# XuehaiPan/mate

Hardware: AMD Instinct MI355X
Metric: env-steps/sec MATE-4v8-9 batch=4096 per GPU (random policy, auto-reset) (higher is better)
Workload: dtype f64; 1 GPU; MATE-4v8-9.yaml batch=4096 envs per GPU, uniform random policy (on-device Philox), fused 256-step launches, restarts every 1 launch(es); global_batch=4096, parallelism=env-shard x1, steps_per_launch=256

## Files before the change

include/mate_engine.h:

```cpp
#ifndef MATE_ENGINE_H
#define MATE_ENGINE_H

#include <stdint.h>

#ifdef __cplusplus
extern "C" {
#endif

#define MATE_ABI_VERSION 1

enum {
    MATE_OK = 0,
    MATE_EINVAL = -1,
    MATE_EHIP = -2,
    MATE_ENOMEM = -3,
    MATE_ESTATE = -4
};

enum { MATE_OBS_F32 = 0, MATE_OBS_F64 = 1 };
enum { MATE_ACT_F32 = 0, MATE_ACT_F64 = 1,
       MATE_ACT_CAMERA_DISCRETE = 0x100, MATE_ACT_TARGET_DISCRETE = 0x200 };

typedef struct mate_config {
    int32_t num_cameras, num_targets, num_obstacles;
// ... 157 lines not shown
    float *scalars_dev;
    void  *final_obs_dev;
} mate_first_rows;
int mate_engine_enable_first_rows(mate_engine *engine, const mate_first_rows *config);

int mate_engine_lut_read(mate_engine *engine, int64_t env, int32_t camera, double *phis_host,
                         double *rhos_host, int32_t capacity, int32_t *count);

int mate_engine_enable_outer_boundary(mate_engine *engine, int32_t *capacity);
int mate_engine_lut_read_outer(mate_engine *engine, int64_t env, int32_t camera, double *phis, double *rhos,
                               int32_t capacity, int32_t *count);
int mate_engine_lut_write_outer(mate_engine *engine, int64_t env, int32_t camera, const double *phis_host,
                                const double *rhos_host, int32_t count);
int mate_engine_soft_coverage(mate_engine *engine, const uint32_t *masks_dev, double *matrix_dev, double *scores_dev, void *stream);
int mate_engine_lut_write(mate_engine *engine, int64_t env, int32_t camera, const double *phis_host,
                          const double *rhos_host, int32_t count);
int mate_engine_rebuild_luts(mate_engine *engine, void *stream);

int mate_engine_idle_steps(mate_engine *engine, int64_t *total);

int mate_engine_kernel_time(mate_engine *engine, int32_t enable, double *avg_ms, int64_t *launches);

int mate_engine_last_flow(const mate_engine *engine);

int mate_engine_set_store_form(mate_engine *engine, int32_t shifted);
int mate_engine_block_alloc(int32_t device, int64_t bytes, void **ptr_out);
int mate_engine_block_free(void *ptr);
int mate_engine_block_probe(int32_t device, void *block, int64_t bytes, int32_t rows_per_step, int32_t row_bytes, void *stream,
                            double *gbytes_per_s);
int mate_engine_set_sub_wave(mate_engine *engine, int32_t enable, int32_t *in_use);
int mate_engine_hbm_probe(int32_t device, const void *src, void *dst, int64_t bytes, int32_t mode, void *stream, double *gbytes_per_s);
int mate_engine_memory_hold(int32_t device, int64_t bytes, void **token_out);
int mate_engine_memory_release(void *token);

#ifdef __cplusplus
}
#endif
#endif
```

mate_amd/_native.py:

```python
import ctypes
import os

__all__ = ['lib', 'load', 'EngineError', 'MateConfig', 'MateLayout', 'MateStepIO', 'MatePolicyTape', 'MateRewardRows', 'MateFragmentRows', 'MateFirstRows', 'LIB_PATH', 'check', 'EXPORTED_SYMBOLS']

LIB_PATH = os.environ.get('MATE_ENGINE_LIB') or os.path.join(os.path.dirname(os.path.abspath(__file__)), 'lib', 'libmate_engine.so')

class EngineError(RuntimeError):

    def __init__(self, code, message):
        super().__init__(f'mate_engine error {code}: {message}')
        self.code = code


class MateConfig(ctypes.Structure):
    _fields_ = [
        ('num_cameras', ctypes.c_int32), ('num_targets', ctypes.c_int32), ('num_obstacles', ctypes.c_int32),
        ('max_episode_steps', ctypes.c_int32), ('sparse_reward', ctypes.c_int32),
        ('num_cargoes_per_target', ctypes.c_int32), ('shuffle_entities', ctypes.c_int32),
        ('targets_start_with_cargoes', ctypes.c_int32),
        ('high_capacity_target_split', ctypes.c_double), ('bounty_factor', ctypes.c_double),
        ('transmittance', ctypes.c_double),
        ('camera_radius', ctypes.c_double), ('camera_min_viewing_angle', ctypes.c_double),
        ('camera_max_sight_range', ctypes.c_double), ('camera_rotation_step', ctypes.c_double),
        ('camera_zooming_step', ctypes.c_double),
# ... 83 lines not shown
    'mate_engine_export_state': (INT, [P, P, P]),
    'mate_engine_import_state': (INT, [P, P, P]),
    'mate_engine_enable_state_rows': (INT, [P, P, I32, P, P]),
    'mate_engine_state_rows': (INT, [P, P, I32, P, P, P]),
    'mate_engine_enable_reward_rows': (INT, [P, ctypes.POINTER(MateRewardRows)]),
    'mate_engine_enable_selection': (INT, [P, I32, P, P, P, P, I32]),
    'mate_engine_disable_selection': (INT, [P]),
    'mate_engine_selection_actions': (INT, [P, ctypes.POINTER(P), ctypes.POINTER(I32)]),
    'mate_engine_step_selected': (INT, [P, IO, TAPE, I32, P]),
    'mate_engine_enable_fragment_rows': (INT, [P, ctypes.POINTER(MateFragmentRows)]),
    'mate_engine_fragment_coefficients': (INT, [P, ctypes.POINTER(P), ctypes.POINTER(I32)]),
    'mate_engine_fragment_rows': (INT, [P, ctypes.POINTER(MateFragmentRows), IO, I32, P]),
    'mate_engine_enable_first_rows': (INT, [P, ctypes.POINTER(MateFirstRows)]),
    'mate_engine_lut_read': (INT, [P, I64, I32, P, P, I32, ctypes.POINTER(I32)]),
    'mate_engine_lut_read_outer': (INT, [P, I64, I32, P, P, I32, ctypes.POINTER(I32)]),
    'mate_engine_enable_outer_boundary': (INT, [P, ctypes.POINTER(I32)]),
    'mate_engine_lut_write': (INT, [P, I64, I32, P, P, I32]),
    'mate_engine_lut_write_outer': (INT, [P, I64, I32, P, P, I32]),
    'mate_engine_soft_coverage': (INT, [P, P, P, P, P]),
    'mate_engine_rebuild_luts': (INT, [P, P]),
    'mate_engine_idle_steps': (INT, [P, ctypes.POINTER(I64)]),
    'mate_engine_kernel_time': (INT, [P, I32, F64P, ctypes.POINTER(I64)]),
    'mate_engine_last_flow': (INT, [P]),
    'mate_engine_block_alloc': (INT, [I32, I64, ctypes.POINTER(P)]),
    'mate_engine_block_free': (INT, [P]),
    'mate_engine_block_probe': (INT, [I32, P, I64, I32, I32, P, F64P]),
    'mate_engine_set_store_form': (INT, [P, I32]),
    'mate_engine_memory_hold': (INT, [I32, I64, ctypes.POINTER(P)]),
    'mate_engine_memory_release': (INT, [P]),
    'mate_engine_hbm_probe': (INT, [I32, P, P, I64, I32, P, F64P]),
    'mate_engine_set_sub_wave': (INT, [P, I32, ctypes.POINTER(I32)]),
}
EXPORTED_SYMBOLS = tuple(PROTOTYPES)

lib = None


def load():
    global lib
    if lib is not None:
        return lib
    if not os.path.exists(LIB_PATH):
        raise ImportError(
            f'{LIB_PATH} is missing: build the HIP engine first (python -m mate_amd.build or '
            f'__graft_entry__.build()).  mate_amd has no CPU fallback.')
    import torch
# ... 79 lines not shown
```

mate_amd/build.py:

```python
import json
import os
import re
import subprocess
import sys

HERE = os.path.dirname(os.path.abspath(__file__))
SRC = os.path.join(HERE, 'csrc', 'mate_engine.hip')
DEPS = [SRC] + [os.path.join(HERE, 'csrc', f) for f in ('engine_kernels.hpp', 'reset_kernels.hpp', 'policy_kernels.hpp', 'aux_kernels.hpp', 'attached_tile.hpp', 'state_rows.hpp', 'reward_rows.hpp', 'fragment_rows.hpp', 'selection_rows.hpp', 'device_math.hpp', 'instrument.hpp',
                                                          'shape_groups.hpp', 'shape_group.inc', 'shape_group.hip', 'engine_host.h',
                                                          'opponent_rows.hpp', 'opponent_kernels.inc', 'opponent_kernels.hip')] + [
    os.path.join(os.path.dirname(HERE), 'include', 'mate_engine.h')]
OUT = os.path.join(HERE, 'lib', 'libmate_engine.so')
FLAGS = ['--offload-arch=gfx950', '-O3', '-std=c++17', '-ffp-contract=off', '-fPIC', '-shared',
         '-mllvm', '-disable-machine-licm']


STAMP = os.path.join(HERE, 'lib', 'build_stamp.json')


def source_digest():
    import hashlib
    h = hashlib.sha256(' '.join(FLAGS).encode())
    for d in DEPS:
        with open(d, 'rb') as fh:
            h.update(os.path.basename(d).encode() + b'\0' + fh.read())
    return h.hexdigest()


def needs_build():
    if not os.path.exists(OUT) or not os.path.exists(STAMP):
        return True
    try:
        with open(STAMP) as fh:
            return json.load(fh).get('sources') != source_digest()
    except (OSError, ValueError):
        return True


RESOURCES = os.path.join(HERE, 'lib', 'kernel_resources.json')
OPPONENT_SRC = os.path.join(HERE, 'csrc', 'opponent_kernels.hip')
OPPONENT_RESOURCES = os.path.join(HERE, 'lib', 'kernel_resources_opponents.json')
_REMARK = re.compile(r'remark:\s+(Function Name|TotalSGPRs|VGPRs|ScratchSize \[bytes/lane\]|Dynamic Stack|Occupancy \[waves/SIMD\]|SGPRs Spill|VGPRs Spill): (\S+)')


def parse_resources(text):
    kernels, current = {}, None
    for key, value in _REMARK.findall(text):
        if key == 'Function Name':
            current = kernels.setdefault(value, {})
        elif current is not None:
            current[key.split(' [')[0]] = value if key == 'Dynamic Stack' else int(value)
    return kernels


N_SHAPE_GROUPS = 6


def _compile_and_link(out, extra=(), verbose=False, remarks=False):
    import concurrent.futures
    hipcc = os.environ.get('HIPCC', '/opt/rocm/bin/hipcc')
    objdir = os.path.join(os.path.dirname(OUT), 'obj', os.path.splitext(os.path.basename(out))[0])
    os.makedirs(objdir, exist_ok=True)
    compile_flags = [f for f in FLAGS if f != '-shared'] + list(extra) + ['-DMATE_SPLIT_BUILD'] + (['-Rpass-analysis=kernel-resource-usage'] if remarks else [])
    units = [(SRC, [], os.path.join(objdir, 'mate_engine.o'))]
    units += [(os.path.join(HERE, 'csrc', 'shape_group.hip'), [f'-DMATE_SHAPE_GROUP={k}'], os.path.join(objdir, f'shape_group_{k}.o')) for k in range(N_SHAPE_GROUPS)]
    units += [(OPPONENT_SRC, [], os.path.join(objdir, 'opponent_kernels.o'))]

    def compile_unit(unit):
        src, defs, obj = unit
        cmd = [hipcc] + compile_flags + defs + ['-c', '-o', obj, src]
        if verbose:
            print(' '.join(cmd), flush=True)
        done = subprocess.run(cmd, stdout=subprocess.PIPE, stderr=subprocess.PIPE, universal_newlines=True)
        return cmd, done

    workers = max(1, min(len(units), int(os.environ.get('MATE_BUILD_JOBS', '0')) or (os.cpu_count() or 2)))
    with concurrent.futures.ThreadPoolExecutor(max_workers=workers) as pool:
        results = list(pool.map(compile_unit, units))
    text, opponent_text = '', ''
    for (src, _, _), (cmd, done) in zip(units, results):
        if done.returncode != 0:
            sys.stderr.write(done.stderr)
            raise subprocess.CalledProcessError(done.returncode, cmd)
        if src == OPPONENT_SRC:
            opponent_text += done.stderr
        else:
            text += done.stderr
    link = [hipcc, '--offload-arch=gfx950', '-shared', '-fPIC', '-o', out] + [u[2] for u in units]
    if verbose:
        print(' '.join(link), flush=True)
    done = subprocess.run(link, stdout=subprocess.PIPE, stderr=subprocess.PIPE, universal_newlines=True)
    if done.returncode != 0:
        sys.stderr.write(done.stderr)
        raise subprocess.CalledProcessError(done.returncode, link)
    return text, opponent_text


def build_engine(force=False, verbose=False):
    if not force and not needs_build():
        return OUT
    os.makedirs(os.path.dirname(OUT), exist_ok=True)
    text, opponent_text = _compile_and_link(OUT, verbose=verbose, remarks=True)
    kernels, opponents = parse_resources(text), parse_resources(opponent_text)
    for path, table in ((RESOURCES, kernels), (OPPONENT_RESOURCES, opponents)):
        with open(path, 'w') as f:
            json.dump(table, f, indent=1, sort_keys=True)
    bad = [k for k, r in list(kernels.items()) + list(opponents.items()) if r.get('ScratchSize', 0) != 0 or r.get('Dynamic Stack') != 'False']
    if bad:
        os.remove(OUT)
        raise RuntimeError('kernels with private scratch memory: ' + ', '.join(bad))
    with open(STAMP, 'w') as f:
        json.dump({'sources': source_digest()}, f)
    return OUT


def build_profiling(verbose=False):
    out = os.path.join(HERE, 'lib', 'libmate_engine_prof.so')
    _compile_and_link(out, extra=['-DMATE_PHASE_CLOCKS'], verbose=verbose)
    return out


def build_tools(verbose=False):
    hipcc = os.environ.get('HIPCC', '/opt/rocm/bin/hipcc')
    tools = os.path.join(os.path.dirname(os.path.dirname(os.path.abspath(__file__))), 'tools')
    built = []
    for name in ('store_roof', 'store_bits', 'store_contig', 'store_vmm', 'region_bw', 'valu_rates', 'chunk_order', 'dispatch_probe', 'va_reuse', 'store_layout'):
        src, out = os.path.join(tools, name + '.hip'), os.path.join(tools, name)
        if not os.path.exists(src) or (os.path.exists(out) and os.path.getmtime(out) >= os.path.getmtime(src)):
            continue
        cmd = [hipcc, '--offload-arch=gfx950', '-O3', '-std=c++17', '-I' + os.path.dirname(SRC), '-o', out, src]
# ... 23 lines not shown
```

mate_amd/csrc/engine_host.h:

```cpp
#pragma once
#include <hip/hip_runtime.h>

#include <cstdint>
#include <string>
#include <utility>
#include <vector>

#include "../../include/mate_engine.h"
#include "reset_kernels.hpp"
#include "reward_rows.hpp"
#include "fragment_rows.hpp"
#include "selection_rows.hpp"
#include "opponent_rows.hpp"
#include "state_rows.hpp"
#include "shape_groups.hpp"

using namespace mate;

constexpr size_t kLdsCeiling = 160 * 1024;

struct Switches {
    bool generic = false;
    bool flow_generic = false;
    int stagger = -1;
    int lut_small_cap = 0;
    bool reset_monolithic = false;
    int rollout_rotate = 1;
    bool no_image = false;
    bool policy_split = false;
    int step_split = -1;
    bool zoom_iterate = false;
    bool step_sub_wave = true;
    int sub_wave_mode = 2;
    bool step_greedy_rollout = false;
    bool pipelined_low_priority = true;
    bool pipelined_serial = false;
};
struct StateRows {
    void *dst = nullptr; bool f64 = false; const void *ab = nullptr; void *d_ab = nullptr, *d_ab_demand = nullptr;
    std::vector<double> demand_table;
    bool on() const { return dst != nullptr; }
};
struct RewardRows {
    bool on = false, f64 = false, soft = false, accumulate = false;
    RewardArgs args{};
    int32_t *d_snapshot = nullptr; double *d_matrix = nullptr, *d_scores = nullptr;
};
struct Selection {
    bool on = false, act_f64 = true;
    SelectionArgs args{};
    double *d_actions = nullptr;
    bool masks_stale = false;
};
struct Opponent {
    int kind = MATE_OPPONENT_GREEDY;
    double *d_final = nullptr;
    bool drifted = false;
};
struct FragmentRows {
// ... 15 lines not shown
    Params p{};
    Params *d_params = nullptr;
    Ptrs g{};
    ResetLds rl{};
    ResetLds rl_small{};
    mate_config cfg{};
    int device = 0;
    int64_t N = 0;
    int parity = 0;
    uint32_t tick = 0;
    int64_t steps_since_reset = 0;
    bool was_reset = false;
    bool dev_tick = false;
    int dev_frames = 1;
    int dev_interval = 1;
    int pending_interval = 0;
    bool pipelined = false;
    int pipe_every = 1, pipe_count = 0;
    hipStream_t side = nullptr;
    hipEvent_t ev_launch = nullptr, ev_reset[2] = {nullptr, nullptr};
    bool reset_in_flight[2] = {false, false};
    size_t step_lds = 0, reset_lds = 0;
    KernelSet k{};
    size_t image_wave_bytes = 0;
    int64_t cus = 256;
    int split_on = 0;
    int last_flow = 0;
    std::vector<void *> allocs;
    bool policy_ready = false;
    PolicyPtrs q{};
    int greedy_team_bits = 0;
    int cam_mode = 0, tgt_mode = 0;
    bool xf_relative = false, xf_cam = false, xf_tgt = false;
    std::vector<double> xf_cam_scale, xf_cam_bias, xf_tgt_scale, xf_tgt_bias;
    uint2 *d_xdesc = nullptr;
    void *d_xab = nullptr;
    Opponent opponent;
    StateRows state; RewardRows reward; Selection selection; FragmentRows fragment; FirstRows first;
    int timing = 0;
    int64_t timing_tick = 0;
    std::vector<std::pair<hipEvent_t, hipEvent_t>> events;
    size_t events_used = 0;
};

struct LaunchPlan {
    StepFn step = nullptr; PolicyFn policy = nullptr;
// ... 10 lines not shown
    if (mode == 0 || e->k.sub_wave <= 1 || !(greedy ? (const void *)e->k.rollout_greedy_sub : (const void *)e->k.rollout_sub[0])) return 1;
    if (mode == 1) return e->k.sub_wave;
    if (e->N < 32 * e->cus) return 1;
    if (!greedy && e->p.Nc * e->p.Nt >= 16) return 1;
    return e->k.sub_wave;
}
static int folded_flow(const mate_engine *e, int mode, const Ptrs &g) {
    const bool common = !e->sw.flow_generic && !g.tape_ct && !g.tape_goal && !g.act_discrete && g.obs_mode == 0 && !g.xdesc && !g.xab &&
                        g.scratch_init && (g.cam_obs || e->p.Nc == 0) && g.tgt_obs && g.scalars;
    if (common && mode == MODE_STEP_RANDOM) return FLOW_RANDOM;
    if (common && mode == MODE_STEP) return FLOW_ACT_F32;
    return FLOW_ANY;
}

static LaunchPlan plan_step(const mate_engine *e, int mode, const Ptrs &g) {
    LaunchPlan pl;
    const int flow = pl.last_flow = folded_flow(e, mode, g);
    pl.E = (mode != MODE_OBSERVE && e->sw.step_sub_wave && !e->p.obs_f64) ? sub_wave_of_launch(e, false) : 1;
    if (pl.E > 1) { pl.step = e->k.rollout_sub[flow]; pl.blocks = blocks_of(e, 4 * pl.E); pl.lds = pl.E * e->step_lds; }
    else if (e->split_on && e->k.split[flow]) { pl.step = e->k.split[flow]; pl.blocks = blocks_of(e, 1); pl.threads = 128; pl.lds = e->step_lds / 4; }
    else { pl.step = e->k.step[flow]; pl.blocks = blocks_of(e, 4); pl.lds = e->step_lds; }
    return pl;
}
static LaunchPlan plan_rollout_random(const mate_engine *e, const Ptrs &g) {
    LaunchPlan pl;
    const int flow = pl.last_flow = folded_flow(e, MODE_STEP_RANDOM, g);
    pl.E = sub_wave_of_launch(e, false);
    pl.blocks = blocks_of(e, 4 * pl.E);
    if (pl.E > 1) { pl.step = e->k.rollout_sub[flow]; pl.lds = pl.E * e->step_lds; }
    else { pl.step = e->k.rollout[flow]; pl.lds = (flow == FLOW_RANDOM && e->k.image) ? 4 * e->image_wave_bytes : e->step_lds; }
    return pl;
}
enum PolicyForm { FORM_ROLLOUT, FORM_ROLLOUT_SUB, FORM_STEP_GREEDY, kPolicyForms };
static LaunchPlan policy_form(const mate_engine *e, int form, int team_caller) {
    const Params &p = e->p;
    LaunchPlan pl;
    pl.policy = form == FORM_STEP_GREEDY ? e->k.step_greedy : form == FORM_ROLLOUT_SUB ? e->k.rollout_greedy_sub : e->k.rollout_greedy;
    pl.last_flow = form == FORM_STEP_GREEDY ? FLOW_STEP_GREEDY : FLOW_GREEDY;
    pl.E = form == FORM_ROLLOUT_SUB ? e->k.sub_wave : 1;
    pl.blocks = blocks_of(e, 4 * pl.E);
    const int slice = form == FORM_STEP_GREEDY ? step_greedy_slice_bytes(e->q.PW, e->q.TW, p.Nc, p.Nt, p.MW, team_caller != 0) : policy_slice_bytes(e->q.PW, p.Nc, p.Nt);
    pl.lds = (size_t)pl.E * (4 * (size_t)p.lds_wave_bytes + 4 * (size_t)slice) + (form != FORM_STEP_GREEDY && pl.E == 1 ? 1024 : 0);
    return pl;
}
static LaunchPlan plan_with_policies(const mate_engine *e, bool per_step, int team_caller) {
    const bool sub = (!per_step || e->sw.step_sub_wave) && sub_wave_of_launch(e, true) > 1 && policy_form(e, FORM_ROLLOUT_SUB, team_caller).fits();
    const bool light = per_step && !sub && e->k.step_greedy && !e->sw.step_greedy_rollout && policy_form(e, FORM_STEP_GREEDY, -1).fits();
    return policy_form(e, sub ? FORM_ROLLOUT_SUB : light ? FORM_STEP_GREEDY : FORM_ROLLOUT, team_caller);
}

struct Tiles { unsigned blocks = 0, threads = 256; size_t lds = 0; int E = 0; };
struct AttachedPlan {
// ... 29 lines not shown
```

mate_amd/csrc/mate_engine.hip:

```cpp
#include <hip/hip_runtime.h>
#include <hip/hip_ext.h>

#include <algorithm>
#include <atomic>
#include <cmath>
#include <cstdarg>
#include <cstdio>
#include <cstdlib>
#include <cstring>
#include <map>
#include <mutex>
#include <random>
#include <string>
#include <vector>

#include "../../include/mate_engine.h"
#include "reset_kernels.hpp"
#include "policy_kernels.hpp"
#include "aux_kernels.hpp"
#include "engine_host.h"

using namespace mate;

static thread_local std::string g_error;
// ... 12 lines not shown
        if (e_ != hipSuccess) { (void)hipGetLastError(); return fail(MATE_EHIP, "%s failed: %s", #expr, hipGetErrorString(e_)); }    \
    } while (0)

#ifndef MATE_SPLIT_BUILD
#define MATE_SHAPE_GROUP 0
#include "shape_group.inc"
#undef MATE_SHAPE_GROUP
#define MATE_SHAPE_GROUP 1
#include "shape_group.inc"
#undef MATE_SHAPE_GROUP
#define MATE_SHAPE_GROUP 2
#include "shape_group.inc"
#undef MATE_SHAPE_GROUP
#define MATE_SHAPE_GROUP 3
#include "shape_group.inc"
#undef MATE_SHAPE_GROUP
#define MATE_SHAPE_GROUP 4
#include "shape_group.inc"
#undef MATE_SHAPE_GROUP
#define MATE_SHAPE_GROUP 5
#include "shape_group.inc"
#undef MATE_SHAPE_GROUP
#include "opponent_kernels.inc"
#endif

static KernelSet pick_kernels(int Nc, int Nt, int No, bool f64, bool generic, bool no_image) {
    KernelSet k;
    if (!generic && (pick_kernels_group0(Nc, Nt, No, f64, no_image, &k) || pick_kernels_group1(Nc, Nt, No, f64, no_image, &k) ||
                     pick_kernels_group2(Nc, Nt, No, f64, no_image, &k) || pick_kernels_group3(Nc, Nt, No, f64, no_image, &k) ||
                     pick_kernels_group4(Nc, Nt, No, f64, no_image, &k) || pick_kernels_group5(Nc, Nt, No, f64, no_image, &k))) {
        k.specialised = 1;
        return k;
    }
    return f64 ? f64_kernels<AnyShape>() : f32_kernels<AnyShape, void, true>(no_image);
}

static Switches read_switches() {
    Switches w;
    auto flag = [](const char *name) { const char *v = getenv(name); return v && atoi(v) != 0; };
    w.generic = flag("MATE_GENERIC");
    w.flow_generic = flag("MATE_FLOW_GENERIC");
    if (const char *v = getenv("MATE_STAGGER")) w.stagger = atoi(v);
    if (const char *v = getenv("MATE_LUT_SMALL_CAP")) w.lut_small_cap = atoi(v);
    w.reset_monolithic = flag("MATE_RESET_MONOLITHIC");
    if (const char *v = getenv("MATE_ROLLOUT_ROTATE")) w.rollout_rotate = atoi(v);
    w.zoom_iterate = flag("MATE_ZOOM_ITERATE");
    w.policy_split = flag("MATE_POLICY_SPLIT");
    w.step_greedy_rollout = flag("MATE_STEP_GREEDY_ROLLOUT");
    w.no_image = flag("MATE_NO_IMAGE");
    if (const char *v = getenv("MATE_STEP_SUBWAVE")) w.step_sub_wave = atoi(v) != 0;
    if (const char *v = getenv("MATE_SUBWAVE")) w.sub_wave_mode = atoi(v) == 0 ? 0 : 1;
    if (const char *v = getenv("MATE_STEP_SPLIT")) w.step_split = atoi(v) != 0;
    if (const char *v = getenv("MATE_PIPELINED_PRIORITY")) w.pipelined_low_priority = atoi(v) != 0;
    w.pipelined_serial = flag("MATE_PIPELINED_SERIAL");
    return w;
}

static void note_stream(mate_engine *e, hipStream_t stream) {
    if (e->launched && stream != e->last_stream) e->multi_stream = true;
    e->last_stream = stream; e->launched = true;
}
static int leave_pipelined(mate_engine *e, hipStream_t stream);
static hipError_t wait_for_launches(mate_engine *e) {
    if (e->pipelined && leave_pipelined(e, e->last_stream) != MATE_OK) return hipErrorUnknown;
    hipError_t err = e->multi_stream ? hipErrorInvalidHandle : hipStreamSynchronize(e->last_stream);
    if (err != hipSuccess) { (void)hipGetLastError(); e->last_stream = nullptr; err = hipDeviceSynchronize(); }
    if (err == hipSuccess) { e->multi_stream = false; e->launched = false; }
    return err;
}

static int enter(mate_engine *e, hipStream_t stream, const char *who = nullptr) {
    { const int rc = leave_pipelined(e, stream); if (rc != MATE_OK) return rc; }
    if (who && !e->was_reset) return fail(MATE_ESTATE, "%s called before reset() (or import_state)", who);
    HIP_TRY(hipSetDevice(e->device));
    return MATE_OK;
}
static int enter_host(mate_engine *e) {
// ... 168 lines not shown
    e->cfg = *cfg;
    e->device = device;
    e->N = num_envs;
    Params &p = e->p;
    fill_shape(p, Nc, Nt, No, cfg->obs_dtype == MATE_OBS_F64);
    p.max_episode_steps = cfg->max_episode_steps; p.sparse_reward = cfg->sparse_reward != 0;
    p.num_cargoes_per_target = cfg->num_cargoes_per_target; p.shuffle = cfg->shuffle_entities != 0;
    p.start_with_cargoes = cfg->targets_start_with_cargoes != 0;
    p.n_high = (int)((double)Nt * std::min(std::max(cfg->high_capacity_target_split, 0.0), 1.0));
    p.tau = std::min(std::max(cfg->transmittance, 0.0), 1.0);
    p.cam_radius = cfg->camera_radius; p.theta_min = cfg->camera_min_viewing_angle; p.rmax = cfg->camera_max_sight_range;
    p.rot = cfg->camera_rotation_step; p.zoom = cfg->camera_zooming_step;
    p.area = cfg->camera_min_viewing_angle * (cfg->camera_max_sight_range * cfg->camera_max_sight_range);
    p.tgt_step = cfg->target_step_size; p.tgt_sight = cfg->target_sight_range;
    p.freight_scale = std::ceil(2000.0 / cfg->target_step_size);
    p.bounty_scale = std::ceil(p.freight_scale * std::max(0.0, cfg->bounty_factor));
    p.reward_scale = p.freight_scale + p.bounty_scale;
    p.max_team_reward = p.reward_scale * cfg->num_cargoes_per_target * Nt;
    p.obs_r_lo = cfg->obstacle_radius_range[0]; p.obs_r_hi = cfg->obstacle_radius_range[1];
    p.seed_lo = (uint32_t)seed; p.seed_hi = (uint32_t)(seed >> 32); p.first_env = (uint32_t)first_env_index;
    e->step_lds = 4 * (size_t)p.lds_wave_bytes;
    e->sw = read_switches();
    e->k = pick_kernels(Nc, Nt, No, p.obs_f64 != 0, e->sw.generic, e->sw.no_image);
    { Params pi = p; fill_shape(pi, Nc, Nt, No, false, true); e->image_wave_bytes = e->k.image ? (size_t)pi.lds_wave_bytes : (size_t)p.lds_wave_bytes; }
    if (p.lds_wave_bytes > 0xffff) { delete e; return fail(MATE_EINVAL, "scenario too large for 16-bit LDS descriptors"); }
    ResetLds &rl = e->rl;
    layout_reset_lds(p, rl, std::max(512, next_pow2(Nc > 0 ? 360 + No * 185 + 1 : 1)));
    e->reset_lds = (size_t)rl.total_bytes;
    setup_two_tier(e);
    if (e->step_lds > kLdsCeiling || e->reset_lds > kLdsCeiling) {
        const size_t a = e->step_lds, b = e->reset_lds;
        delete e;
        return fail(MATE_EINVAL, "scenario too large for the 160 KiB LDS (%zu / %zu bytes)", a, b);
    }

    int rc = MATE_OK;
    const size_t N = (size_t)num_envs;
    Ptrs &g = e->g;
    g.N = num_envs;
    {
        hipDeviceProp_t prop;
        const int64_t cus = hipGetDeviceProperties(&prop, device) == hipSuccess ? prop.multiProcessorCount : 256;
        e->cus = cus;
        const int digits = e->sw.stagger >= 0 ? e->sw.stagger : 0;

        if (e->sw.step_split < 0) e->sw.step_split = (Nc > 0 && num_envs <= 8 * cus) ? 1 : 0;
// ... 35 lines not shown
            g.scratch_init = d;
            return MATE_OK;
        });
        if (rc) break;
        std::vector<double> ranges((size_t)(Nc + No + Nt) * 4, 0.0);
        if (Nc) std::memcpy(ranges.data(), cfg->camera_location_ranges, sizeof(double) * 4 * Nc);
        if (No) std::memcpy(ranges.data() + 4 * Nc, cfg->obstacle_location_ranges, sizeof(double) * 4 * No);
        std::memcpy(ranges.data() + 4 * (Nc + No), cfg->target_location_ranges, sizeof(double) * 4 * Nt);
        double *d_ranges = nullptr;
        if ((rc = dev_alloc(e, &d_ranges, ranges.size()))) break;
        if (hipMemcpy(d_ranges, ranges.data(), ranges.size() * 8, hipMemcpyHostToDevice) != hipSuccess) { rc = fail(MATE_EHIP, "range upload failed"); break; }
        g.reset_ranges = d_ranges;
    } while (0);
    if (rc == MATE_OK) rc = dev_alloc(e, &e->d_params, (size_t)1);
    if (rc == MATE_OK) g.dev_tick_ptr = reinterpret_cast<uint32_t *>(reinterpret_cast<char *>(e->d_params) + offsetof(Params, dev_tick));
    if (rc == MATE_OK && hipMemcpy(e->d_params, &e->p, sizeof(Params), hipMemcpyHostToDevice) != hipSuccess) rc = fail(MATE_EHIP, "params upload failed");
    if (rc == MATE_OK) {
        const KernelSet &k = e->k;
        hipError_t err = hipSuccess;
        auto opt_in = [&](auto fn, size_t bytes) { if (err == hipSuccess) err = set_dynamic_lds(fn, bytes); };
        for (int f = 0; f < 3; ++f) opt_in(k.step[f], e->step_lds);
        for (int f = 0; f < 2; ++f) opt_in(k.rollout[f], f == 1 && k.image ? 4 * e->image_wave_bytes : e->step_lds);
        for (int f = 0; f < 3; ++f) opt_in(k.rollout_sub[f], k.sub_wave * e->step_lds);
        with_obs_type(p.obs_f64 != 0, [&](auto tag) { opt_in(&reset_kernel<decltype(tag)>, e->reset_lds); });
        if (err != hipSuccess) rc = fail(MATE_EHIP, "hipFuncSetAttribute failed: %s", hipGetErrorString(err));
    }
    if (rc != MATE_OK) { mate_engine_destroy(e); return rc; }
    *out = e;
    return MATE_OK;
}

extern "C" int mate_engine_destroy(mate_engine *e) {
    if (!e) return MATE_OK;
    (void)hipSetDevice(e->device);
    if (e->side) {
        (void)hipStreamSynchronize(e->side);
        (void)hipStreamDestroy(e->side);
        if (e->ev_launch) (void)hipEventDestroy(e->ev_launch);
        for (int q = 0; q < 2; ++q) if (e->ev_reset[q]) (void)hipEventDestroy(e->ev_reset[q]);
    }
    for (auto &ev : e->events) { (void)hipEventDestroy(ev.first); (void)hipEventDestroy(ev.second); }
    for (void *ptr : e->allocs) (void)hipFree(ptr);
    delete e;
    return MATE_OK;
}

// ... 743 lines not shown
extern "C" int mate_engine_step(mate_engine *e, const mate_step_io *io, int32_t auto_reset, void *stream) {
    return attached_last(e, launch_step(e, io, MODE_STEP, auto_reset, (hipStream_t)stream), (hipStream_t)stream);
}
extern "C" int mate_engine_step_random(mate_engine *e, const mate_step_io *io, int32_t auto_reset, void *stream) {
    return attached_last(e, launch_step(e, io, MODE_STEP_RANDOM, auto_reset, (hipStream_t)stream), (hipStream_t)stream);
}
static int rollout_random_impl(mate_engine *e, const mate_step_io *io, int32_t steps, int32_t auto_reset, void *stream_) {
    if (!e) return fail(MATE_EINVAL, "null engine");
    hipStream_t stream = (hipStream_t)stream_;
    { const int rc_ = enter(e, stream, "rollout"); if (rc_ != MATE_OK) return rc_; }
    if (e->dev_tick) return fail(MATE_ESTATE, "not available while the step counter is device-resident (mate_engine_device_tick)");
    if (steps < 1) return fail(MATE_EINVAL, "rollout needs at least one step");
    { const int rc_ = check_attached_call(e, io, false, false); if (rc_ != MATE_OK) return rc_; }
    note_stream(e, stream);
    { int rc = flush_pending(e, auto_reset, kRolloutFlow, stream); if (rc != MATE_OK) return rc; }
    Ptrs g = e->g;
    apply_io(g, io);
    g.mode = MODE_STEP_RANDOM; g.parity = e->parity; g.reset_kind = -1; g.tick = e->tick; g.rollout_steps = steps;
    g.tape_ct = nullptr; g.tape_goal = nullptr;
    g.rotate_prio = e->sw.rollout_rotate;
    if (auto_reset != 1) g.done_count = nullptr;
    Timed t;
    { const int rc_ = take_timing_events(e, true, &t); if (rc_ != MATE_OK) return rc_; }
    const LaunchPlan pl = plan_rollout_random(e, g);
    e->last_flow = pl.last_flow;
    hipExtLaunchKernelGGL(pl.step, dim3(pl.blocks), dim3(pl.threads), pl.lds, stream, t.a, t.b, 0, (const Params *)e->d_params, (const Ptrs)g);
    HIP_TRY(hipGetLastError());
    e->tick += (uint32_t)steps;
    { const int rc_ = attached_behind_step(e, false, io, steps, stream); if (rc_ != MATE_OK) return rc_; }
    if (auto_reset >= 1) e->selection.masks_stale = true;
    return restart_finished(e, auto_reset, Restart{nullptr, false, RESET_FLAGGED, PH_PLACE | PH_LUT, false, false, 0u, kRolloutFlow}, stream);
}

extern "C" int mate_engine_rollout_random(mate_engine *e, const mate_step_io *io, int32_t steps, int32_t auto_reset, void *stream) {
    return attached_last(e, rollout_random_impl(e, io, steps, auto_reset, stream), (hipStream_t)stream);
}

static int policy_enable(mate_engine *e) {
    if (e->policy_ready) return MATE_OK;
    const Params &p = e->p;
    PolicyPtrs &q = e->q;
    q.TW = pol_target_words(p.Nt);
    q.PW = pol_record_words(p.Nc, p.Nt);
    q.caller_team = -1;
    q.memory_period = 25;
    q.noise_scale = 0.5;
    q.lds_bytes = round_up((q.PW + policy_staging_words(p.Nc, p.Nt) + p.SW + p.DW) * 8 + p.MW * 4 + 4, 16);
// ... 447 lines not shown
extern "C" int mate_engine_debug_phase_clocks(mate_engine *e, long long *buf_dev) {
    if (!e) return fail(MATE_EINVAL, "null engine");
    e->g.phase_clocks = buf_dev;
    return MATE_OK;
}
extern "C" int mate_engine_debug_skip(mate_engine *e, int32_t mask) {
    if (!e) return fail(MATE_EINVAL, "null engine");
    e->g.debug_skip = mask;
    return MATE_OK;
}

extern "C" int mate_engine_idle_steps(mate_engine *e, int64_t *total) {
    if (!e || !total) return fail(MATE_EINVAL, "null argument");
    { const int rc_ = enter_host(e); if (rc_ != MATE_OK) return rc_; }
    std::vector<int32_t> host((size_t)e->N);
    HIP_TRY(hipMemcpy(host.data(), e->g.idle_steps, sizeof(int32_t) * host.size(), hipMemcpyDeviceToHost));
    int64_t sum = 0;
    for (int32_t v : host) sum += v;
    *total = sum;
    return MATE_OK;
}

extern "C" int mate_engine_last_flow(const mate_engine *e) { return e ? e->last_flow : MATE_EINVAL; }

extern "C" int mate_engine_set_store_form(mate_engine *e, int32_t shifted) {
    if (!e) return fail(MATE_EINVAL, "null engine");
    e->g.store_shifted = shifted ? 1 : 0;
    return MATE_OK;
}

namespace {
struct ScatteredBlock { int device; size_t bytes; std::vector<hipMemGenericAllocationHandle_t> chunks; };
std::mutex g_blocks_mutex;
std::map<void *, ScatteredBlock> g_blocks;
std::atomic<int64_t> g_dead_range_bytes{0};
constexpr size_t kBlockChunk = (size_t)2 << 20;
}

extern "C" int mate_engine_block_alloc(int32_t device, int64_t bytes, void **ptr_out) {
    if (!ptr_out || bytes <= 0) return fail(MATE_EINVAL, "block_alloc: null output or empty block");
    *ptr_out = nullptr;
    HIP_TRY(hipSetDevice(device));
    hipMemAllocationProp prop = {};
    prop.type = hipMemAllocationTypePinned;
    prop.location.type = hipMemLocationTypeDevice;
    prop.location.id = device;
// ... 246 lines not shown
```

mate_amd/engine.py:

```python
import ctypes
import os
import time
import warnings

import numpy as np
import torch

from mate_amd import _native, constants as consts, spaces
from mate_amd._native import MateConfig, MateFirstRows, MateFragmentRows, MateLayout, MatePolicyTape, MateRewardRows, MateStepIO, check
from mate_amd.auxiliary_rewards import REWARD_REDUCTIONS, reward_coefficient_table, reward_term_keys
from mate_amd.config import scenario_tables

__all__ = ['Engine', 'EngineGroups', 'Stepper', 'export_layout', 'reward_coefficient_table', 'encode_selection', 'decode_selection',
           'SCALAR_NAMES', 'REWARD_REDUCTIONS', 'TARGET_AGENTS']

SCALAR_NAMES = ('camera_team_reward', 'target_team_reward', 'done', 'coverage_rate', 'real_coverage_rate',
                'mean_transport_rate', 'num_delivered_cargoes', 'normalized_target_team_reward')


def export_layout(Nc, Nt, No):
    fields = [
        ('cam_x', (Nc,)), ('cam_y', (Nc,)), ('obs_x', (No,)), ('obs_y', (No,)), ('obs_radius', (No,)),
        ('tgt_capacity', (Nt,)), ('camera_obstacle_view_mask', (Nc, No)),
        ('cam_phi', (Nc,)), ('cam_theta', (Nc,)), ('tgt_x', (Nt,)), ('tgt_y', (Nt,)),
# ... 780 lines not shown
        check(self.lib.mate_engine_snapshot_episode_stats(self._h, ctypes.c_void_p(out.data_ptr()), self._stream()))
        return out

    def set_sub_wave(self, enable='auto'):
        in_use = ctypes.c_int32()
        check(self.lib.mate_engine_set_sub_wave(self._h, 2 if enable == 'auto' else int(bool(enable)), ctypes.byref(in_use)))
        return in_use.value

    @property
    def sub_wave(self):
        in_use = ctypes.c_int32()
        check(self.lib.mate_engine_set_sub_wave(self._h, -1, ctypes.byref(in_use)))
        return in_use.value

    def kernel_time(self, enable=1):
        avg, n = ctypes.c_double(), ctypes.c_int64()
        check(self.lib.mate_engine_kernel_time(self._h, int(enable), ctypes.byref(avg), ctypes.byref(n)))
        return avg.value, n.value

    @property
    def last_flow(self):
        return int(self.lib.mate_engine_last_flow(self._h))

    def unpack_masks(self, masks=None, words_host=None):
        words = (words_host if words_host is not None else (self.masks if masks is None else masks).cpu().numpy()).astype(np.uint32)
        N, Nc, Nt, No = self.num_envs, self.num_cameras, self.num_targets, self.num_obstacles
        bits = ((words[:, :, None] >> np.arange(32, dtype=np.uint32)) & 1).astype(bool).reshape(N, -1)
        L = self.layout
        NJ = Nc + No + Nt
        ct = bits[:, L.bit_camera_target:L.bit_camera_target + Nc * Nt].reshape(N, Nc, Nt)
        cc = bits[:, L.bit_camera_camera:L.bit_camera_camera + Nc * Nc].reshape(N, Nc, Nc)
        rows = bits[:, L.bit_target_row:L.bit_target_row + Nt * NJ].reshape(N, Nt, NJ)
        co = np.zeros((N, Nc, No), dtype=bool)
        for c in range(Nc):
            co[:, c] = bits[:, L.bit_camera_obstacle + 64 * c:L.bit_camera_obstacle + 64 * c + No]
        return {
            'camera_target_view_mask': ct, 'camera_camera_view_mask': cc,
            'target_camera_view_mask': rows[:, :, :Nc], 'target_obstacle_view_mask': rows[:, :, Nc:Nc + No],
            'target_target_view_mask': rows[:, :, Nc + No:], 'camera_obstacle_view_mask': co,
            'tracked_bits': ct.any(axis=1),
        }


class Stepper:

    def __init__(self, eng, cam_act, tgt_act, auto_reset=True, graph_steps=0, between=None, versus=None, frame_skip=1):
# ... 176 lines not shown
```

Measured before the change: 757.5 million env-steps/s.

## Add dedicated image rollout kernel with wave priority rotation for random flow

Adds a separate image-layout rollout kernel for the random-policy flow. It is compiled in its own unit for a fixed list of shapes, launched with bounds of 256 threads and 4 blocks, and selected when sub-wave is off. The kernel sets a per-step wave priority with s_setprio, using a rotating, lag-based or load-based scheme, so that the four waves in a block make progress together. It also records per-wave progress in LDS. The separate compilation unit may change register allocation, and the priority games may or may not cut tail stalls between the waves.

```diff
diff --git a/include/mate_engine.h b/include/mate_engine.h
--- a/include/mate_engine.h
+++ b/include/mate_engine.h
@@ -203,6 +203,7 @@
 int mate_engine_kernel_time(mate_engine *engine, int32_t enable, double *avg_ms, int64_t *launches);
 
 int mate_engine_last_flow(const mate_engine *engine);
+int mate_engine_rollout_successor(const mate_engine *engine);
 
 int mate_engine_set_store_form(mate_engine *engine, int32_t shifted);
 int mate_engine_block_alloc(int32_t device, int64_t bytes, void **ptr_out);
diff --git a/mate_amd/_native.py b/mate_amd/_native.py
--- a/mate_amd/_native.py
+++ b/mate_amd/_native.py
@@ -129,6 +129,7 @@
     'mate_engine_idle_steps': (INT, [P, ctypes.POINTER(I64)]),
     'mate_engine_kernel_time': (INT, [P, I32, F64P, ctypes.POINTER(I64)]),
     'mate_engine_last_flow': (INT, [P]),
+    'mate_engine_rollout_successor': (INT, [P]),
     'mate_engine_block_alloc': (INT, [I32, I64, ctypes.POINTER(P)]),
     'mate_engine_block_free': (INT, [P]),
     'mate_engine_block_probe': (INT, [I32, P, I64, I32, I32, P, F64P]),
diff --git a/mate_amd/build.py b/mate_amd/build.py
--- a/mate_amd/build.py
+++ b/mate_amd/build.py
@@ -8,7 +8,8 @@
 SRC = os.path.join(HERE, 'csrc', 'mate_engine.hip')
 DEPS = [SRC] + [os.path.join(HERE, 'csrc', f) for f in ('engine_kernels.hpp', 'reset_kernels.hpp', 'policy_kernels.hpp', 'aux_kernels.hpp', 'attached_tile.hpp', 'state_rows.hpp', 'reward_rows.hpp', 'fragment_rows.hpp', 'selection_rows.hpp', 'device_math.hpp', 'instrument.hpp',
                                                           'shape_groups.hpp', 'shape_group.inc', 'shape_group.hip', 'engine_host.h',
-                                                          'opponent_rows.hpp', 'opponent_kernels.inc', 'opponent_kernels.hip')] + [
+                                                          'opponent_rows.hpp', 'opponent_kernels.inc', 'opponent_kernels.hip',
+                                                          'image_rollout.hpp', 'image_rollout.hip')] + [
     os.path.join(os.path.dirname(HERE), 'include', 'mate_engine.h')]
 OUT = os.path.join(HERE, 'lib', 'libmate_engine.so')
 FLAGS = ['--offload-arch=gfx950', '-O3', '-std=c++17', '-ffp-contract=off', '-fPIC', '-shared',
@@ -40,6 +41,8 @@
 RESOURCES = os.path.join(HERE, 'lib', 'kernel_resources.json')
 OPPONENT_SRC = os.path.join(HERE, 'csrc', 'opponent_kernels.hip')
 OPPONENT_RESOURCES = os.path.join(HERE, 'lib', 'kernel_resources_opponents.json')
+ROLLOUT_SRC = os.path.join(HERE, 'csrc', 'image_rollout.hip')
+ROLLOUT_RESOURCES = os.path.join(HERE, 'lib', 'kernel_resources_rollout.json')
 _REMARK = re.compile(r'remark:\s+(Function Name|TotalSGPRs|VGPRs|ScratchSize \[bytes/lane\]|Dynamic Stack|Occupancy \[waves/SIMD\]|SGPRs Spill|VGPRs Spill): (\S+)')
 
 
@@ -64,7 +67,7 @@
     compile_flags = [f for f in FLAGS if f != '-shared'] + list(extra) + ['-DMATE_SPLIT_BUILD'] + (['-Rpass-analysis=kernel-resource-usage'] if remarks else [])
     units = [(SRC, [], os.path.join(objdir, 'mate_engine.o'))]
     units += [(os.path.join(HERE, 'csrc', 'shape_group.hip'), [f'-DMATE_SHAPE_GROUP={k}'], os.path.join(objdir, f'shape_group_{k}.o')) for k in range(N_SHAPE_GROUPS)]
-    units += [(OPPONENT_SRC, [], os.path.join(objdir, 'opponent_kernels.o'))]
+    units += [(OPPONENT_SRC, [], os.path.join(objdir, 'opponent_kernels.o')), (ROLLOUT_SRC, [], os.path.join(objdir, 'image_rollout.o'))]
 
     def compile_unit(unit):
         src, defs, obj = unit
@@ -77,13 +80,15 @@
     workers = max(1, min(len(units), int(os.environ.get('MATE_BUILD_JOBS', '0')) or (os.cpu_count() or 2)))
     with concurrent.futures.ThreadPoolExecutor(max_workers=workers) as pool:
         results = list(pool.map(compile_unit, units))
-    text, opponent_text = '', ''
+    text, opponent_text, rollout_text = '', '', ''
     for (src, _, _), (cmd, done) in zip(units, results):
         if done.returncode != 0:
             sys.stderr.write(done.stderr)
             raise subprocess.CalledProcessError(done.returncode, cmd)
         if src == OPPONENT_SRC:
             opponent_text += done.stderr
+        elif src == ROLLOUT_SRC:
+            rollout_text += done.stderr
         else:
             text += done.stderr
     link = [hipcc, '--offload-arch=gfx950', '-shared', '-fPIC', '-o', out] + [u[2] for u in units]
@@ -93,19 +98,19 @@
     if done.returncode != 0:
         sys.stderr.write(done.stderr)
         raise subprocess.CalledProcessError(done.returncode, link)
-    return text, opponent_text
+    return text, opponent_text, rollout_text
 
 
 def build_engine(force=False, verbose=False):
     if not force and not needs_build():
         return OUT
     os.makedirs(os.path.dirname(OUT), exist_ok=True)
-    text, opponent_text = _compile_and_link(OUT, verbose=verbose, remarks=True)
-    kernels, opponents = parse_resources(text), parse_resources(opponent_text)
-    for path, table in ((RESOURCES, kernels), (OPPONENT_RESOURCES, opponents)):
+    text, opponent_text, rollout_text = _compile_and_link(OUT, verbose=verbose, remarks=True)
+    kernels, opponents, rollouts = parse_resources(text), parse_resources(opponent_text), parse_resources(rollout_text)
+    for path, table in ((RESOURCES, kernels), (OPPONENT_RESOURCES, opponents), (ROLLOUT_RESOURCES, rollouts)):
         with open(path, 'w') as f:
             json.dump(table, f, indent=1, sort_keys=True)
-    bad = [k for k, r in list(kernels.items()) + list(opponents.items()) if r.get('ScratchSize', 0) != 0 or r.get('Dynamic Stack') != 'False']
+    bad = [k for k, r in list(kernels.items()) + list(opponents.items()) + list(rollouts.items()) if r.get('ScratchSize', 0) != 0 or r.get('Dynamic Stack') != 'False']
     if bad:
         os.remove(OUT)
         raise RuntimeError('kernels with private scratch memory: ' + ', '.join(bad))
diff --git a/mate_amd/csrc/engine_host.h b/mate_amd/csrc/engine_host.h
--- a/mate_amd/csrc/engine_host.h
+++ b/mate_amd/csrc/engine_host.h
@@ -14,6 +14,7 @@
 #include "opponent_rows.hpp"
 #include "state_rows.hpp"
 #include "shape_groups.hpp"
+#include "image_rollout.hpp"
 
 using namespace mate;
 
@@ -35,6 +36,8 @@
     bool step_greedy_rollout = false;
     bool pipelined_low_priority = true;
     bool pipelined_serial = false;
+    bool rollout_successor = true;
+    int rollout_prio = kPrioRotate;
 };
 struct StateRows {
     void *dst = nullptr; bool f64 = false; const void *ab = nullptr; void *d_ab = nullptr, *d_ab_demand = nullptr;
@@ -96,6 +99,7 @@
     bool reset_in_flight[2] = {false, false};
     size_t step_lds = 0, reset_lds = 0;
     KernelSet k{};
+    StepFn image_rollout = nullptr;
     size_t image_wave_bytes = 0;
     int64_t cus = 256;
     int split_on = 0;
@@ -152,12 +156,15 @@
     else { pl.step = e->k.step[flow]; pl.blocks = blocks_of(e, 4); pl.lds = e->step_lds; }
     return pl;
 }
-static LaunchPlan plan_rollout_random(const mate_engine *e, const Ptrs &g) {
+static LaunchPlan plan_rollout_random(const mate_engine *e, const Ptrs &g, bool *successor = nullptr) {
     LaunchPlan pl;
     const int flow = pl.last_flow = folded_flow(e, MODE_STEP_RANDOM, g);
     pl.E = sub_wave_of_launch(e, false);
     pl.blocks = blocks_of(e, 4 * pl.E);
-    if (pl.E > 1) { pl.step = e->k.rollout_sub[flow]; pl.lds = pl.E * e->step_lds; }
+    const bool succ = pl.E == 1 && flow == FLOW_RANDOM && e->k.image && e->image_rollout;
+    if (successor) *successor = succ;
+    if (succ) { pl.step = e->image_rollout; pl.lds = image_rollout_lds_bytes(e->image_wave_bytes); }
+    else if (pl.E > 1) { pl.step = e->k.rollout_sub[flow]; pl.lds = pl.E * e->step_lds; }
     else { pl.step = e->k.rollout[flow]; pl.lds = (flow == FLOW_RANDOM && e->k.image) ? 4 * e->image_wave_bytes : e->step_lds; }
     return pl;
 }
diff --git a/mate_amd/csrc/image_rollout.hip b/mate_amd/csrc/image_rollout.hip
--- /dev/null
+++ b/mate_amd/csrc/image_rollout.hip
@@ -0,0 +1,15 @@
+#include <hip/hip_runtime.h>
+#include "image_rollout.hpp"
+
+namespace mate {
+
+#define MATE_IMAGE_ROLLOUT_SHAPES(X) X(4, 8, 9) X(4, 8, 0) X(0, 8, 32) X(4, 2, 9) X(4, 4, 9) X(4, 4, 0)
+
+StepFn pick_image_rollout(int Nc, int Nt, int No) {
+#define X(C, T, O) if (Nc == C && Nt == T && No == O) return (StepFn)image_rollout_kernel<FixedShape<C, T, O, false, true>>;
+    MATE_IMAGE_ROLLOUT_SHAPES(X)
+#undef X
+    return nullptr;
+}
+
+}
diff --git a/mate_amd/csrc/image_rollout.hpp b/mate_amd/csrc/image_rollout.hpp
--- /dev/null
+++ b/mate_amd/csrc/image_rollout.hpp
@@ -0,0 +1,179 @@
+#pragma once
+#include "engine_kernels.hpp"
+
+namespace mate {
+
+enum RolloutPrio : int { kPrioNone = 0, kPrioRotate = 1, kPrioLag = 2, kPrioHeavy = 3, kPrioLast = 3 };
+constexpr uint32_t kProgressFinished = 0x7fffffffu;
+constexpr size_t image_rollout_lds_bytes(size_t image_wave_bytes) { return 4 * image_wave_bytes + 16; }
+
+constexpr int kHeavyPairs = 9, kLightPairs = 4;
+typedef uint32_t progress_words __attribute__((ext_vector_type(4)));
+typedef __attribute__((address_space(3))) volatile uint32_t lds_progress_word;
+typedef __attribute__((address_space(3))) volatile progress_words lds_progress_words;
+__device__ __forceinline__ void publish_progress(uint32_t progress, int wave, uint32_t step) { *(lds_progress_word *)(uintptr_t)(progress + 4u * (uint32_t)wave) = step; }
+
+__device__ __forceinline__ void set_wave_prio(int level) {
+    if (level & 2) { if (level & 1) __builtin_amdgcn_s_setprio(3); else __builtin_amdgcn_s_setprio(2); }
+    else { if (level & 1) __builtin_amdgcn_s_setprio(1); else __builtin_amdgcn_s_setprio(0); }
+}
+__device__ __forceinline__ int lag_bias(uint32_t progress, int wave, int step) {
+    publish_progress(progress, wave, (uint32_t)step);
+    const progress_words w = *(lds_progress_words *)(uintptr_t)progress;
+    int ahead_of_me = 0, behind_me = 0;
+#pragma unroll
+    for (int i = 0; i < 4; ++i) {
+        const int other = __builtin_amdgcn_readfirstlane((int)w[i]);
+        ahead_of_me += other > step;
+        behind_me += other < step;
+    }
+    return ahead_of_me == 3 ? 1 : behind_me == 3 ? -1 : 0;
+}
+__device__ __forceinline__ int biased_level(int rot, int bias) { return bias > 0 ? rot | 2 : bias < 0 ? rot & 1 : rot; }
+
+template <typename Shape>
+__global__ __launch_bounds__(256, 4) void image_rollout_kernel(const Params *__restrict__ pp, const Ptrs g) {
+    using ObsT = float;
+    constexpr int FLOW = FLOW_RANDOM;
+    static_assert(Shape::kImage && Shape::kHoldRoles, "the row-image shapes: held lane roles");
+    static_assert(kNearWords == kRoleRounds, "one ballot per range round");
+    const Shape shape(pp, true);
+    const Params &p = shape.get();
+    extern __shared__ __align__(16) unsigned char smem[];
+    if (blockIdx.x == 0 && threadIdx.x == 0 && g.done_count) g.done_count[g.parity ^ 1] = 0;
+    const int wave = __builtin_amdgcn_readfirstlane((int)(threadIdx.x >> 6));
+    const int lane = threadIdx.x & 63;
+    const int64_t env = (int64_t)blockIdx.x * 4 + wave;
+    if (env >= g.N) {
+        publish_progress(lds_addr(smem + 4 * p.lds_wave_bytes), wave, kProgressFinished);
+        return;
+    }
+    const Ptrs &gk = kernarg_ptrs(g);
+    MATE_PROF(const long long t_wave = (long long)__builtin_amdgcn_s_memtime();)
+    {
+        Ctx<ObsT> c(p, gk, smem + wave * p.lds_wave_bytes, lane, env, FLOW_ANY);
+        load_records(c);
+        wave_sync();
+        build_entities(c);
+        list_finished_at_entry(c);
+        wave_sync();
+    }
+    PROLOGUE_STAMP(8);
+    RangeRoles roles;
+    {
+        Ctx<ObsT> c(p, gk, smem + wave * p.lds_wave_bytes, lane, env, FLOW);
+        range_roles(c, roles);
+        pin_roles(roles);
+        PROLOGUE_STAMP(9);
+        image_statics(c);
+    }
+    PROLOGUE_STAMP(10);
+    NearCarry near{};
+    {
+        Ctx<ObsT> c(p, gk, smem + wave * p.lds_wave_bytes, lane, env, FLOW);
+        near_seed(c, roles, near);
+    }
+    uint32_t hw_id;
+    asm volatile("s_getreg_b32 %0, hwreg(HW_REG_HW_ID)" : "=s"(hw_id));
+    const int wave_slot = (int)(hw_id & 15u);
+    MATE_PROF(long long acc[8] = {0, 0, 0, 0, 0, 0, 0, 0};
+              long long t_prev = (long long)__builtin_amdgcn_s_memtime();
+              const long long t_first = t_prev, r_first = (long long)__builtin_amdgcn_s_memrealtime();)
+    bool stepped = false;
+    int last_gw = -1;
+    int heavy = 0;
+    DrawCarry carry{0u, 0u, 0xffffffffu};
+    DrawRole draws_of_lane;
+    {
+        Ctx<ObsT> c(p, gk, smem + wave * p.lds_wave_bytes, lane, env, FLOW);
+        draws_of_lane = draw_role(c);
+    }
+    HeldState h{};
+    int finished = 0;
+    const uint32_t tick0 = g.tick;
+    const uint32_t cam_low = (uint32_t)(reinterpret_cast<uintptr_t>(g.cam_obs) >> 4) & 7u, tgt_low = (uint32_t)(reinterpret_cast<uintptr_t>(g.tgt_obs) >> 4) & 7u;
+    const int n_steps = g.rollout_steps;
+    {
+        Ctx<ObsT> c(p, gk, smem + wave * p.lds_wave_bytes, lane, env, FLOW);
+        held_load(c, h);
+        finished = __builtin_amdgcn_readfirstlane((int)(c.ei(EI_DONE) != 0));
+    }
+    PROLOGUE_STAMP(11);
+#pragma clang loop unroll(disable)
+    for (int r = 0; r < n_steps; ++r) {
+        int lane_r = lane, wave_r = wave;
+        asm volatile("" : "+v"(lane_r));
+        asm volatile("" : "+s"(wave_r));
+        const Params *pr = pp;
+        asm volatile("" : "+s"(pr));
+        const Shape shape_r(pr, true);
+        const Params &p = shape_r.get();
+        const int64_t env_r = (int64_t)blockIdx.x * 4 + wave_r;
+        pin_roles(roles, p.range_rounds, true, p.sector_rounds == 1);
+        Ctx<ObsT> c(p, gk, smem + wave_r * p.lds_wave_bytes, lane_r, env_r, FLOW);
+        c.out = (int64_t)r * g.N + env_r;
+        c.statics_done = stepped;
+        c.pivots = Shape::kGreedyHeld;
+        const int prio = g.rotate_prio;
+        int bias = 0;
+        if (prio == kPrioLag) bias = lag_bias(lds_addr(smem + 4 * p.lds_wave_bytes), wave_r, r);
+        if (finished != 0) {
+            if (lane_r == 0 && g.scalars) write_idle_row(g.scalars + c.out * 8);
+            if (lane_r == 0 && g.idle_steps) g.idle_steps[env_r] += 1;
+            continue;
+        }
+        const uint32_t tick = tick0 + (uint32_t)r;
+        if (prio == kPrioRotate) set_wave_prio((r + wave_slot) & 3);
+        else if (prio != kPrioNone) {
+            if (prio == kPrioHeavy) bias = heavy >= kHeavyPairs ? 1 : heavy <= kLightPairs ? -1 : 0;
+            set_wave_prio(biased_level((r + wave_slot) & 3, bias));
+        }
+        ROLL_STAMP(7);
+        StepDraws draws{0.0, 0.0};
+        pin_draw_role(draws_of_lane);
+        draws = step_draws(c, tick, &carry, &draws_of_lane);
+        ROLL_STAMP(0);
+        simulate_cameras_held(c, draws, h);
+        ROLL_STAMP(1);
+        simulate_targets_held(c, draws, near, h);
+        ROLL_STAMP(2);
+        uint32_t seen = 0u;
+        unsigned long long sector_ballot = 0ull;
+        update_view<true, true>(c, tick, S_TRANSMIT, true, roles, seen, &near, &sector_ballot);
+        bool tracked; int inside;
+        view_tail_held(c, sector_ballot, h, tracked, inside);
+        heavy = __popcll(sector_ballot);
+        ROLL_STAMP(3);
+        finished = assign_and_score_held(c, tick, g.scalars, h, tracked, inside);
+        ROLL_STAMP(4);
+        image_targets_held(c, h, last_gw); image_blocks(c, roles, seen);
+        ROLL_STAMP(5);
+        image_store(c, cam_low, tgt_low); store_masks(c);
+        wave_sync();
+        stepped = true;
+        ROLL_STAMP(6);
+    }
+    publish_progress(lds_addr(smem + 4 * p.lds_wave_bytes), wave, kProgressFinished);
+    MATE_PROF(if (lane == 0 && g.phase_clocks)
+                  for (int i = 0; i < 8; ++i) g.phase_clocks[env * kClockStride + i] = acc[i];
+              if (lane == 0 && g.phase_clocks) {
+                  uint32_t hwid, xccid;
+                  asm volatile("s_getreg_b32 %0, hwreg(HW_REG_HW_ID)" : "=s"(hwid));
+                  asm volatile("s_getreg_b32 %0, hwreg(HW_REG_XCC_ID)" : "=s"(xccid));
+                  g.phase_clocks[env * kClockStride + 13] = ((long long)xccid << 32) | (long long)hwid;
+                  g.phase_clocks[env * kClockStride + 14] = (long long)__builtin_amdgcn_s_memtime() - t_first;
+                  g.phase_clocks[env * kClockStride + 15] = (long long)__builtin_amdgcn_s_memrealtime() - r_first;
+              }
+              const long long t_epilogue = (long long)__builtin_amdgcn_s_memtime();)
+    {
+        Ctx<ObsT> c(p, gk, smem + wave * p.lds_wave_bytes, lane, env, FLOW_ANY);
+        held_store(c, h);
+        store_dynamic(c);
+    }
+    MATE_PROF(if (lane == 0 && g.phase_clocks) g.phase_clocks[env * kClockStride + 12] = (long long)__builtin_amdgcn_s_memtime() - t_epilogue;)
+}
+
+using StepFn = void (*)(const Params *, const Ptrs);
+StepFn pick_image_rollout(int Nc, int Nt, int No);
+
+}
diff --git a/mate_amd/csrc/mate_engine.hip b/mate_amd/csrc/mate_engine.hip
--- a/mate_amd/csrc/mate_engine.hip
+++ b/mate_amd/csrc/mate_engine.hip
@@ -58,6 +58,7 @@
 #include "shape_group.inc"
 #undef MATE_SHAPE_GROUP
 #include "opponent_kernels.inc"
+#include "image_rollout.hip"
 #endif
 
 static KernelSet pick_kernels(int Nc, int Nt, int No, bool f64, bool generic, bool no_image) {
@@ -89,6 +90,8 @@
     if (const char *v = getenv("MATE_STEP_SPLIT")) w.step_split = atoi(v) != 0;
     if (const char *v = getenv("MATE_PIPELINED_PRIORITY")) w.pipelined_low_priority = atoi(v) != 0;
     w.pipelined_serial = flag("MATE_PIPELINED_SERIAL");
+    if (const char *v = getenv("MATE_ROLLOUT_SUCCESSOR")) w.rollout_successor = atoi(v) != 0;
+    if (const char *v = getenv("MATE_ROLLOUT_PRIO")) { const int m = atoi(v); if (m >= kPrioNone && m <= kPrioLast) w.rollout_prio = m; }
     return w;
 }
 
@@ -303,6 +306,7 @@
     e->step_lds = 4 * (size_t)p.lds_wave_bytes;
     e->sw = read_switches();
     e->k = pick_kernels(Nc, Nt, No, p.obs_f64 != 0, e->sw.generic, e->sw.no_image);
+    if (e->k.image && e->sw.rollout_successor) e->image_rollout = pick_image_rollout(Nc, Nt, No);
     { Params pi = p; fill_shape(pi, Nc, Nt, No, false, true); e->image_wave_bytes = e->k.image ? (size_t)pi.lds_wave_bytes : (size_t)p.lds_wave_bytes; }
     if (p.lds_wave_bytes > 0xffff) { delete e; return fail(MATE_EINVAL, "scenario too large for 16-bit LDS descriptors"); }
     ResetLds &rl = e->rl;
@@ -384,6 +388,7 @@
         for (int f = 0; f < 3; ++f) opt_in(k.step[f], e->step_lds);
         for (int f = 0; f < 2; ++f) opt_in(k.rollout[f], f == 1 && k.image ? 4 * e->image_wave_bytes : e->step_lds);
         for (int f = 0; f < 3; ++f) opt_in(k.rollout_sub[f], k.sub_wave * e->step_lds);
+        opt_in(e->image_rollout, image_rollout_lds_bytes(e->image_wave_bytes));
         with_obs_type(p.obs_f64 != 0, [&](auto tag) { opt_in(&reset_kernel<decltype(tag)>, e->reset_lds); });
         if (err != hipSuccess) rc = fail(MATE_EHIP, "hipFuncSetAttribute failed: %s", hipGetErrorString(err));
     }
@@ -1173,7 +1178,9 @@
     if (auto_reset != 1) g.done_count = nullptr;
     Timed t;
     { const int rc_ = take_timing_events(e, true, &t); if (rc_ != MATE_OK) return rc_; }
-    const LaunchPlan pl = plan_rollout_random(e, g);
+    bool successor = false;
+    const LaunchPlan pl = plan_rollout_random(e, g, &successor);
+    if (successor) g.rotate_prio = e->sw.rollout_rotate ? e->sw.rollout_prio : kPrioNone;
     e->last_flow = pl.last_flow;
     hipExtLaunchKernelGGL(pl.step, dim3(pl.blocks), dim3(pl.threads), pl.lds, stream, t.a, t.b, 0, (const Params *)e->d_params, (const Ptrs)g);
     HIP_TRY(hipGetLastError());
@@ -1667,6 +1674,15 @@
 }
 
 extern "C" int mate_engine_last_flow(const mate_engine *e) { return e ? e->last_flow : MATE_EINVAL; }
+extern "C" int mate_engine_rollout_successor(const mate_engine *e) {
+    if (!e) return MATE_EINVAL;
+    Ptrs g = e->g;
+    g.tape_ct = nullptr; g.tape_goal = nullptr;
+    if (!g.cam_obs) g.cam_obs = (void *)e; if (!g.tgt_obs) g.tgt_obs = (void *)e; if (!g.scalars) g.scalars = (float *)e;
+    bool successor = false;
+    (void)plan_rollout_random(e, g, &successor);
+    return successor ? 1 : 0;
+}
 
 extern "C" int mate_engine_set_store_form(mate_engine *e, int32_t shifted) {
     if (!e) return fail(MATE_EINVAL, "null engine");
diff --git a/mate_amd/engine.py b/mate_amd/engine.py
--- a/mate_amd/engine.py
+++ b/mate_amd/engine.py
@@ -826,6 +826,10 @@
     def last_flow(self):
         return int(self.lib.mate_engine_last_flow(self._h))
 
+    @property
+    def rollout_successor(self):
+        return int(self.lib.mate_engine_rollout_successor(self._h)) == 1
+
     def unpack_masks(self, masks=None, words_host=None):
         words = (words_host if words_host is not None else (self.masks if masks is None else masks).cpu().numpy()).astype(np.uint32)
         N, Nc, Nt, No = self.num_envs, self.num_cameras, self.num_targets, self.num_obstacles
```

Measured after the change: 738.6 million env-steps/s. 2.5% lower.
